# ChrisDud0257/SSL

Measured on AMD Instinct MI355X. Metric: SSG-loss edge-pixels/sec (fwd+bwd) 3x256x256 k_s=25 k_w=9, higher is better.
Workload: dtype f32; 1 GPU; C2: batch 16 x 3x256x256 per GPU, Laplacian mask, k_s=25 k_w=9 sigma=1.0, L1+KL w=1e3, SSGs materialised; launch=per-kernel, ranks_seen=1, edge_px_rank0=76466, images_rank0=16, input_checksum=c1391ff6908574f6, gradient_accumulation=fixed-point integer atomics (bit-reproducible, the shipped default), prewarm_steps=1949, parallelism=images sharded x1, no data-path collective

## Files before the change

### ssl_amd/csrc/ssg_dense.hip

```cpp
#include "ssg_host.hpp"

namespace ssg {

typedef float f2 __attribute__((ext_vector_type(2)));

template <int D>
__device__ __forceinline__ float quad_next(float v) {
  constexpr int ctrl = D == 1 ? 0xF9 : 0xFE;
  return __builtin_bit_cast(float, __builtin_amdgcn_update_dpp(0, __builtin_bit_cast(int, v), ctrl, 0xf, 0xf, true));
}

template <int LO, int LEN, typename T, int N>
__device__ __forceinline__ T block_sum(const T (&e)[N]) {
  static_assert(LEN >= 1 && (LEN & (LEN - 1)) == 0 && LO >= 0 && LO + LEN <= N, "power-of-two block inside the array");
  if constexpr (LEN == 1) return e[LO];
  else return block_sum<LO, LEN / 2>(e) + block_sum<LO + LEN / 2, LEN / 2>(e);
}
constexpr int floor_pow2(int n) { return n < 2 ? 1 : 2 * floor_pow2(n / 2); }
template <int LO, int LEN, typename T, int N>
__device__ __forceinline__ T sum_from(const T (&e)[N]) {
  constexpr int B = floor_pow2(LEN);
  if constexpr (B == LEN) return block_sum<LO, LEN>(e);
  else return block_sum<LO, B>(e) + sum_from<LO + B, LEN - B>(e);
}
template <int HI, int LEN, typename T, int N>
__device__ __forceinline__ T sum_upto(const T (&e)[N]) {
  constexpr int B = floor_pow2(LEN);
  if constexpr (B == LEN) return block_sum<HI - LEN, LEN>(e);
  else return block_sum<HI - B, B>(e) + sum_upto<HI - B, LEN - B>(e);
}

template <int KW>
__device__ __forceinline__ float tap_sum(const float (&v)[KW], const float (&w)[KW], float rest) {
  static_assert(KW % 2 == 1 && KW >= 5, "pairs of taps and a last one");
  constexpr int NP = KW / 2;
  f2 a = f2{v[0], v[1]} * f2{w[0], w[1]}, b = f2{v[2], v[3]} * f2{w[2], w[3]};
#pragma unroll
  for (int j = 2; j < NP; ++j) {
    const f2 vv = f2{v[2 * j], v[2 * j + 1]}, ww = f2{w[2 * j], w[2 * j + 1]};
    if (j % 2 == 0) a = __builtin_elementwise_fma(vv, ww, a);
    else b = __builtin_elementwise_fma(vv, ww, b);
  }
  const f2 r2 = a + b;
  return (r2.x + r2.y) + __builtin_fmaf(w[KW - 1], v[KW - 1], rest);
}

constexpr int DT_X = 32;
constexpr int dense_lane_px(int kw) { return kw == 9 ? 10 : 12; }
constexpr bool dense_h_paired(int kw) { return kw == 9; }
constexpr int dense_h_group(int kw) { return kw == 9 ? 10 : 12; }
constexpr int dense_h_stride(int kw) { return kw == 9 ? 40 : 49; }
__device__ __forceinline__ int dense_h_col(int ex, int L, int G, bool paired) {
  const int k = ex % L;
  return paired ? G * (ex / L) + 2 * (k % (L / 2)) + k / (L / 2) : ex;
}

template <int KS, int KW, int C, int NW, bool TM = false, bool RAW = false, int NCH = 0>
__device__ __forceinline__ void fwd_dense_body(const DenseParams &p) {
  static_assert(!(TM && RAW), "raw distances go to the caller's row-major rows");
  constexpr int NT = 64 * NW;
  constexpr int HP = KS / 2, HK = KW / 2, P = KS * KS, HALO = HP + HK, DT_Y = 16 - 2 * HK;
  constexpr int RH = DT_Y + 2 * HALO, RWD = DT_X + 2 * HALO, RS = RWD + 1;
  constexpr int UH = DT_Y + 2 * HK, UW = DT_X + 2 * HK;
  constexpr int L = dense_lane_px(KW), HL = L / 2;
  constexpr int NV = HL + KW - 1;
  constexpr int DT_HS = dense_h_stride(KW);
  constexpr bool HPAIR = dense_h_paired(KW);
  constexpr int HG = dense_h_group(KW);
  constexpr int NE_MAX = DT_Y * DT_X, NCHUNK = NCH > 0 ? NCH : NE_MAX / 64;
  constexpr bool PIPE = dense_h_paired(KW) && NCH > 0 && NCH <= 2 && !TM;
  static_assert(NCH == 0 || (dense_h_paired(KW) && NCH * 64 <= NE_MAX), "chunk classes exist for the 8 x 32 tiles only");
  static_assert(!TM || !HPAIR, "tile-major rows use the k_w 13 pixel map");
  static_assert(UH == 16 && DT_X == 32 && 4 * L >= UW && 3 * HG + L <= DT_HS && HG >= L && (HPAIR || HG == L) && L % 2 == 0 && KW - 1 <= L,
                "lane map: 16 U-rows x 4 column groups (one quad) of L pixels; a window spans two lanes");

  extern __shared__ __attribute__((aligned(16))) float smem[];
  float *reg = smem;
  float *F = reg + C * RH * RS;
  float *HF = F + UH * UW;
  float *Hb = HF + UH * DT_HS;
  double *rsum = (double *)Hb;
  constexpr int RSTR = UH * DT_HS / 2;
  static_assert(NE_MAX <= RSTR, "row sums alias the wave's H buffer");
  int *elist = (int *)(Hb + NW * UH * DT_HS);
  int *misc = elist + NE_MAX * 3;

  const int tid = threadIdx.x, lane = tid & 63, wv = tid >> 6;
  const int tslot = blockIdx.x / p.nimg, which = blockIdx.x - tslot * p.nimg;
  if (tslot >= dense_tile_count(p.n_dense)) return;
  if (p.tm_slots > 0 && tm_active(p.n_dense, p.tm_slots, rows_to_do(p.n_dev, p.n_host)) != TM) return;
  if (TM && p.tm_slots <= 0) return;
  if (p.n_dense[1] != DT_Y) {
    if (p.status && tid == 0) atomicOr(p.status, 1);
    return;
  }
  const int H = p.H, W = p.W;
  const int tx_n = (W + DT_X - 1) / DT_X, ty_n = (H + DT_Y - 1) / DT_Y;
  const int listed = dense_tile_at(p.n_dense, p.tiles, p.B * ty_n * tx_n, tslot);
  if (TM && p.strips && (listed & TILE_IN_STRIP)) return;
  if constexpr (NCH > 0) {
    if (((listed & TILE_HUGE) != 0) != (NCH > 2)) return;
  }
  const int tile = dense_tile_id(listed);
  const int b = tile / (tx_n * ty_n), tr = tile - b * tx_n * ty_n;
  const int ty0 = (tr / tx_n) * DT_Y, tx0 = (tr % tx_n) * DT_X;
  const int nrows = rows_to_do(p.n_dev, p.n_host);

  constexpr int CPLF = (RWD + 15) / 16, RPP = NT / 16, NPASS = (C * RH + RPP - 1) / RPP;
  const int lx = tid % 16, lr = tid / 16;
  int rank_px = -1;
  if constexpr (HPAIR) {
    const int y = ty0 + tid / DT_X, x = tx0 + tid % DT_X;
    const int v = p.rank[((size_t)b * H + (y < H ? y : H - 1)) * W + (x < W ? x : W - 1)];
    rank_px = (y < H && x < W) ? v : -1;
  }
  float rv[NPASS][CPLF];
  int rdst[NPASS];
  {
    const float *src = p.img[which] + (size_t)b * C * H * W;
#pragma unroll
    for (int h = 0; h < NPASS; ++h) {
      const int R = h * RPP + lr;
      const bool on = R < C * RH;
      const int Rc = on ? R : 0;
      const int c = Rc / RH, ry = Rc - c * RH;
      int gy = reflect_idx(ty0 - HALO + ry, H);
      gy = gy < 0 ? 0 : (gy >= H ? H - 1 : gy);
      const float *srow = src + ((size_t)c * H + gy) * W;
      rdst[h] = on ? (c * RH + ry) * RS : -1;
#pragma unroll
      for (int k = 0; k < CPLF; ++k) {
        int gx = reflect_idx(tx0 - HALO + lx + 16 * k, W);
        gx = gx < 0 ? 0 : (gx >= W ? W - 1 : gx);
        rv[h][k] = srow[gx];
      }
    }
  }
  if constexpr (HPAIR) {
    static_assert(DT_Y * DT_X == NT, "one thread per tile pixel");
    int *wcnt = misc + 16, *bstart = wcnt + NW * 32;
    const int ey = tid / DT_X, ex = tid % DT_X;
    int r = rank_px;
    if (r >= nrows) r = -1;
    elist[3 * tid + 2] = -1;
    const int bank = (DT_HS * ey + dense_h_col(ex, L, HG, true)) & 31;
    int pib = 0, mycnt = 0;
    for (int bk = 0; bk < 32; ++bk) {
      const unsigned long long m = __ballot(r >= 0 && bank == bk);
      if (bank == bk) pib = __popcll(m & ((1ull << lane) - 1ull));
      if (lane == bk) mycnt = __popcll(m);
    }
    if (lane < 32) wcnt[wv * 32 + lane] = mycnt;
    __syncthreads();
    if (tid < 32) {
      int c[NW], tot = 0;
#pragma unroll
      for (int k = 0; k < NW; ++k) {
        c[k] = wcnt[k * 32 + tid];
        tot += c[k];
      }
      int incl = tot;
#pragma unroll
      for (int o = 1; o < 32; o <<= 1) {
        const int t = __shfl_up(incl, o, 32);
        if (tid >= o) incl += t;
      }
      int run = incl - tot;
#pragma unroll
      for (int k = 0; k < NW; ++k) {
        bstart[k * 32 + tid] = run;
        run += c[k];
      }
      if (tid == 31) misc[NW] = 32 * ((incl + 31) / 32);
    }
    __syncthreads();
    if (r >= 0) {
      const int ng = misc[NW] / 32, i = bstart[wv * 32 + bank] + pib;
      const int pos = (i % ng) * 32 + i / ng;
      elist[3 * pos + 0] = ey;
      elist[3 * pos + 1] = ex;
      elist[3 * pos + 2] = r;
    }
  } else {
    static_assert(HPAIR || (DT_Y == 4 && NCHUNK == 2), "pair map: 4 x 32 tile, two pixels per lane");
    if (tid < NE_MAX) {
      const int pp = tid >> 6, ln = tid & 63;
      const int ey = 2 * (ln >> 5) + pp, ex = ln & 31;
      const int y = ty0 + ey, x = tx0 + ex;
      int r = (y < H && x < W) ? p.rank[((size_t)b * H + y) * W + x] : -1;
      if (r >= nrows) r = -1;
      elist[3 * tid + 0] = ey;
      elist[3 * tid + 1] = ex;
      elist[3 * tid + 2] = r;
    }
    if (tid == 0) misc[NW] = NE_MAX;
  }
#pragma unroll
  for (int h = 0; h < NPASS; ++h)
#pragma unroll
    for (int k = 0; k < CPLF; ++k)
      if (rdst[h] >= 0 && lx + 16 * k < RWD) reg[rdst[h] + lx + 16 * k] = rv[h][k];
  __syncthreads();
  const int n_e = misc[NW];
  for (int i = tid; i < UH * UW; i += NT) {
    const int ur = i / UW, uc = i - ur * UW;
    float t = 0.f;
#pragma unroll
    for (int c = 0; c < C; ++c) {
      const float v = reg[(c * RH + ur + HP) * RS + uc + HP];
      t = __builtin_fmaf(v, v, t);
    }
    F[i] = t;
  }
  __syncthreads();
  for (int i = tid; i < UH * DT_X; i += NT) {
    const int ur = i / DT_X, tc = i - ur * DT_X;
    float t = 0.f;
#pragma unroll
    for (int kx = 0; kx < KW; ++kx) t += F[ur * UW + tc + kx];
    HF[ur * DT_HS + dense_h_col(tc, L, HG, HPAIR)] = t;
  }
  __syncthreads();

  const int r = lane >> 2, g = lane & 3;
  f2 iu[C][HL];
#pragma unroll
  for (int c = 0; c < C; ++c)
#pragma unroll
    for (int j = 0; j < HL; ++j) {
      const float *q = reg + (c * RH + r + HP) * RS + L * g + HP + j;
      iu[c][j] = f2{q[0], q[HL]};
    }
  f2 Fv[NV];
#pragma unroll
  for (int m = 0; m < NV; ++m) {
    const int c0 = L * g + m, c1 = c0 + HL;
    Fv[m] = f2{F[r * UW + (c0 < UW ? c0 : UW - 1)], F[r * UW + (c1 < UW ? c1 : UW - 1)]};
  }
  float *hb = Hb + wv * UH * DT_HS;
  float *hrow = hb + r * DT_HS + HG * g;
  const float nk = (float)(-1.4426950408889634 / ((double)(C * KW * KW) * (double)p.sigma));
  double rs[NCHUNK];
#pragma unroll
  for (int k = 0; k < NCHUNK; ++k) rs[k] = 0.0;
  float *outp = p.out[which];
  int hoff[NCHUNK];
  size_t orow[NCHUNK];
  bool eon[NCHUNK];
#pragma unroll
  for (int ck = 0; ck < NCHUNK; ++ck) {
    const int e = ck * 64 + lane;
    eon[ck] = e < n_e && elist[3 * (e < n_e ? e : 0) + 2] >= 0;
    const int ec = (eon[ck] || !HPAIR) ? e : 0;
    const int ey = elist[3 * ec], ex = elist[3 * ec + 1];
    hoff[ck] = ey * DT_HS + dense_h_col(ex, L, HG, HPAIR);
    orow[ck] = eon[ck] ? (size_t)elist[3 * ec + 2] * P : 0;
  }

  const int n_e_stage = SSG_DBG(p, 2) ? 0 : n_e;
  const bool do_store = !SSG_DBG(p, 1);
  constexpr int SB = (KS == 49 && !TM) ? 7 : 13;
  constexpr int REM = (NCHUNK <= 2) ? KS % NW : 0;
  static_assert(REM == 0 || (REM == 1 && NW == 4 && KS > SB && KS <= 2 * SB), "one shared row, four runs: two store groups halved");
  constexpr int RUN1 = (SB + 1) / 2, RUN3 = SB + (KS - SB) / 2;
  const int wvu = __builtin_amdgcn_readfirstlane(wv);
  const int run_lo = wvu == 0 ? 0 : wvu == 1 ? RUN1 : wvu == 2 ? SB : RUN3;
  const int run_hi = wvu == 0 ? RUN1 : wvu == 1 ? SB : wvu == 2 ? RUN3 : KS;
  auto do_row = [&](const int qyi, auto shared_c, auto nact_c) {
    constexpr bool shared_row = decltype(shared_c)::value;
    constexpr int NACT = decltype(nact_c)::value;
    const int ylo = (-HK > -qyi) ? -HK : -qyi, yhi = (HK < KS - 1 - qyi) ? HK : KS - 1 - qyi;
    float wgt[KW];
#pragma unroll
    for (int k = 0; k < KW; ++k) wgt[k] = (k - HK >= ylo && k - HK <= yhi) ? 1.f : 0.f;
    const bool interior = ylo == -HK && yhi == HK;
    float av[NCHUNK];
#pragma unroll
    for (int ck = 0; ck < NCHUNK; ++ck) {
      av[ck] = 0.f;
      if (ck * 64 < n_e && (ylo > -HK || yhi < HK)) {
        const float *fc = HF + hoff[ck];
        float fv[KW], cw[KW];
#pragma unroll
        for (int k = 0; k < KW; ++k) {
          fv[k] = fc[k * DT_HS];
          cw[k] = 1.f - wgt[k];
        }
        av[ck] = tap_sum<KW>(fv, cw, 0.f);
      }
    }
    const float *rq = reg + (r + qyi) * RS + L * g;
    f2 w[C][HL];
    auto fill_window = [&](auto sc) {
      constexpr int S0 = decltype(sc)::value;
#pragma unroll
      for (int c = 0; c < C; ++c)
#pragma unroll
        for (int a = 0; a < L; ++a) {
          const float v = rq[c * RH * RS + ((a - S0) % L + L) % L + S0];
          if (a < HL) w[c][a].x = v;
          else w[c][a - HL].y = v;
        }
    };
    if constexpr (!shared_row) {
      fill_window(std::integral_constant<int, 0>{});
    } else {
      if (run_lo == 0) fill_window(std::integral_constant<int, 0>{});
      else if (run_lo == RUN1) fill_window(std::integral_constant<int, RUN1>{});
      else if (run_lo == SB) fill_window(std::integral_constant<int, SB>{});
      else fill_window(std::integral_constant<int, RUN3>{});
    }
    float evb[TM ? 1 : NCHUNK][TM ? 1 : SB];
    float *tmq = nullptr;
    if constexpr (TM) tmq = p.tm[which] + ((size_t)tslot * P + (size_t)qyi * KS) * (size_t)NE_MAX + lane;
    float hvp[PIPE ? NCHUNK : 1][KW];
    auto step = [&](auto qc, auto split_c) {
      constexpr int qxi = decltype(qc)::value;
      constexpr bool SPLIT = decltype(split_c)::value;
      constexpr int xlo = (-HK > -qxi) ? -HK : -qxi, xhi = (HK < KS - 1 - qxi) ? HK : KS - 1 - qxi;
      f2 E[HL];
      if constexpr (NCHUNK <= 2) {
#pragma unroll
        for (int c = 0; c < C; ++c) {
#pragma unroll
          for (int j = 0; j < HL; ++j) {
            const int a = (j + qxi) % L;
            const f2 wv2 = a < HL ? w[c][a] : w[c][a - HL].yx;
            const f2 d = iu[c][j] - wv2;
            E[j] = c == 0 ? d * d : __builtin_elementwise_fma(d, d, E[j]);
          }
        }
      } else {
#pragma unroll
        for (int j = 0; j < HL; ++j) {
          const int a = (j + qxi) % L;
          f2 t = f2{0.f, 0.f};
#pragma unroll
          for (int c = 0; c < C; ++c) {
            const f2 wv2 = a < HL ? w[c][a] : w[c][a - HL].yx;
            const f2 d = iu[c][j] - wv2;
            t = __builtin_elementwise_fma(d, d, t);
          }
          E[j] = t;
        }
      }
      f2 Hs[HL];
      if constexpr (xlo == -HK && xhi == HK) {
        float Pf[L], Sf[L];
        static_for(std::make_integer_sequence<int, HL>{}, [&](auto mc) {
          constexpr int m = decltype(mc)::value;
          const f2 pl = sum_from<0, m + 1>(E);
          const f2 su = sum_upto<HL, HL - m>(E);
          const f2 tot = sum_from<0, HL>(E);
          Pf[m] = pl.x;
          Pf[m + HL] = tot.x + pl.y;
          Sf[m + HL] = su.y;
          Sf[m] = su.x + tot.y;
        });
        float hs[L];
        if constexpr (KW == 9 && L == 10) {
          hs[0] = Pf[KW - 1];
#pragma unroll
          for (int k = 1; k < L; ++k) hs[k] = Sf[k];
          asm volatile("s_nop 1\n\t"
                       "v_add_f32_dpp %0, %8, %0 quad_perm:[1,2,3,3] row_mask:0xf bank_mask:0xf bound_ctrl:1\n\t"
                       "v_add_f32_dpp %1, %9, %1 quad_perm:[1,2,3,3] row_mask:0xf bank_mask:0xf bound_ctrl:1\n\t"
                       "v_add_f32_dpp %2, %10, %2 quad_perm:[1,2,3,3] row_mask:0xf bank_mask:0xf bound_ctrl:1\n\t"
                       "v_add_f32_dpp %3, %11, %3 quad_perm:[1,2,3,3] row_mask:0xf bank_mask:0xf bound_ctrl:1\n\t"
                       "v_add_f32_dpp %4, %12, %4 quad_perm:[1,2,3,3] row_mask:0xf bank_mask:0xf bound_ctrl:1\n\t"
                       "v_add_f32_dpp %5, %13, %5 quad_perm:[1,2,3,3] row_mask:0xf bank_mask:0xf bound_ctrl:1\n\t"
                       "v_add_f32_dpp %6, %14, %6 quad_perm:[1,2,3,3] row_mask:0xf bank_mask:0xf bound_ctrl:1\n\t"
                       "v_add_f32_dpp %7, %15, %7 quad_perm:[1,2,3,3] row_mask:0xf bank_mask:0xf bound_ctrl:1"
                       : "+v"(hs[2]), "+v"(hs[3]), "+v"(hs[4]), "+v"(hs[5]), "+v"(hs[6]), "+v"(hs[7]), "+v"(hs[8]), "+v"(hs[9])
                       : "v"(Pf[0]), "v"(Pf[1]), "v"(Pf[2]), "v"(Pf[3]), "v"(Pf[4]), "v"(Pf[5]), "v"(Pf[6]), "v"(Pf[7]));
        } else {
        static_for(std::make_integer_sequence<int, L>{}, [&](auto kc) {
          constexpr int k = decltype(kc)::value, last = k + KW - 1;
          if constexpr (last < L) {
            static_assert(k == 0 || last == L - 1, "in-lane windows: a prefix or a suffix");
            hs[k] = k == 0 ? Pf[last] : Sf[k];
          } else {
            hs[k] = Sf[k] + quad_next<1>(Pf[last - L]);
          }
        });
        }
#pragma unroll
        for (int k = 0; k < HL; ++k) Hs[k] = f2{hs[k], hs[k + HL]};
      } else {
        f2 V[NV];
#pragma unroll
        for (int m = 0; m < NV; ++m) {
          if (m < HL) V[m] = E[m];
          else if (m < L) V[m] = f2{E[m - HL].y, quad_next<1>(E[m - HL].x)};
          else V[m] = f2{quad_next<1>(E[m - L].x), quad_next<1>(E[m - L].y)};
        }
#pragma unroll
        for (int k = 0; k < HL; ++k) {
          f2 t = f2{0.f, 0.f};
          bool first = true;
#pragma unroll
          for (int tp = 0; tp < KW; ++tp) {
            const bool kept = tp - HK >= xlo && tp - HK <= xhi;
            const f2 v = kept ? V[k + tp] : Fv[k + tp];
            t = first ? v : t + v;
            first = false;
          }
          Hs[k] = t;
        }
      }
      if constexpr (HPAIR) {
#pragma unroll
        for (int k = 0; k < HL; ++k) *(f2 *)(hrow + 2 * k) = Hs[k];
      } else {
#pragma unroll
        for (int k = 0; k < HL; ++k) {
          hrow[k] = Hs[k].x;
          hrow[k + HL] = Hs[k].y;
        }
      }
      if (qxi + 1 < KS) {
        constexpr int sl = qxi % L;
#pragma unroll
        for (int c = 0; c < C; ++c) {
          const float v = rq[c * RH * RS + L + qxi];
          if constexpr (sl < HL) w[c][sl].x = v;
          else w[c][sl - HL].y = v;
        }
      }
      float dpair[2];
      if constexpr (!HPAIR) {
        if (n_e_stage > 0) {
          const float *hc = hb + hoff[0];
          float hv[KW + 1];
#pragma unroll
          for (int k = 0; k <= KW; ++k) hv[k] = hc[k * DT_HS];
          if (interior) {
            f2 t01 = f2{hv[2], hv[3]} + f2{hv[4], hv[5]}, t23 = f2{hv[6], hv[7]} + f2{hv[8], hv[9]};
            t01 = t01 + f2{hv[10], hv[11]};
            t01 = t01 + t23;
            const float common = (t01.x + t01.y) + (hv[1] + hv[KW - 1]);
            dpair[0] = common + hv[0];
            dpair[1] = common + hv[KW];
          } else {
            float h0[KW], h1[KW];
#pragma unroll
            for (int k = 0; k < KW; ++k) {
              h0[k] = hv[k];
              h1[k] = hv[k + 1];
            }
            dpair[0] = tap_sum<KW>(h0, wgt, av[0]);
            dpair[1] = tap_sum<KW>(h1, wgt, av[1]);
          }
        }
      }
      auto edge_gather = [&](int ck, float (&hv)[KW]) {
        const float *hc = hb + hoff[ck];
#pragma unroll
        for (int k = 0; k < KW; ++k) hv[k] = hc[k * DT_HS];
      };
      auto edge_emit = [&](auto qe_c, int ck, float d) {
        constexpr int QE = decltype(qe_c)::value;
          float ev;
          if constexpr (RAW) {
            ev = d;
          } else {
            ev = __builtin_amdgcn_exp2f(d * nk);
            rs[ck] += (double)ev;
            asm volatile("" : "+v"(rs[ck]));
          }
          if constexpr (TM) {
            if (do_store) tmq[QE * NE_MAX + ck * 64] = ev;
          } else {
          evb[ck][QE % SB] = ev;
          if (eon[ck] && do_store) {
            float *o = outp + orow[ck] + qyi * KS;
            constexpr bool ends = SPLIT ? (QE + 1 == RUN1 || QE + 1 == SB || QE + 1 == RUN3 || QE + 1 == KS)
                                        : (QE % SB == SB - 1 || QE == KS - 1);
            if constexpr (ends) {
              constexpr int q0 = !SPLIT ? QE - QE % SB : (QE + 1 == RUN1 ? 0 : QE + 1 == SB ? RUN1 : QE + 1 == RUN3 ? SB : RUN3);
              constexpr int cnt = QE + 1 - q0, i0 = q0 % SB;
#pragma unroll
              for (int t = 0; t + 4 <= cnt; t += 4) {
                float4 v4 = make_float4(evb[ck][i0 + t], evb[ck][i0 + t + 1], evb[ck][i0 + t + 2], evb[ck][i0 + t + 3]);
                if constexpr (RAW) {
                  float4 old;
                  __builtin_memcpy(&old, o + q0 + t, 16);
                  v4.x += old.x; v4.y += old.y; v4.z += old.z; v4.w += old.w;
                }
                __builtin_memcpy(o + q0 + t, &v4, 16);
              }
#pragma unroll
              for (int t = cnt & ~3; t < cnt; ++t) {
                if constexpr (RAW) o[q0 + t] += evb[ck][i0 + t];
                else o[q0 + t] = evb[ck][i0 + t];
              }
            }
          }
          }
      };
#pragma unroll
      for (int ck = 0; ck < (NACT >= 0 ? NACT : NCHUNK); ++ck) {
        if (NACT >= 0 || ck * 64 < n_e_stage) {
          if constexpr (PIPE && !SPLIT) {
            if constexpr (qxi > 0) edge_emit(std::integral_constant<int, qxi - 1>{}, ck, tap_sum<KW>(hvp[ck], wgt, av[ck]));
            edge_gather(ck, hvp[ck]);
            if constexpr (qxi == KS - 1) edge_emit(std::integral_constant<int, KS - 1>{}, ck, tap_sum<KW>(hvp[ck], wgt, av[ck]));
          } else if constexpr (HPAIR) {
            float hv[KW];
            edge_gather(ck, hv);
            edge_emit(std::integral_constant<int, qxi>{}, ck, tap_sum<KW>(hv, wgt, av[ck]));
          } else {
            edge_emit(std::integral_constant<int, qxi>{}, ck, dpair[ck]);
          }
        }
      }
    };
    if constexpr (!shared_row) {
      static_for(std::make_integer_sequence<int, KS>{}, [&](auto qc) { step(qc, std::false_type{}); });
    } else {
      static_for(std::make_integer_sequence<int, KS>{}, [&](auto qc) {
        constexpr int qxi = decltype(qc)::value;
        if (qxi >= run_lo && qxi < run_hi) step(qc, std::true_type{});
      });
    }
  };
  if (!SSG_DBG(p, 64)) {
#define SSG_ALL_ROWS(NACT_)                                                                                    \
  do {                                                                                                         \
    _Pragma("unroll 1") for (int qyi = wv; qyi < KS - REM; qyi += NW)                                          \
        do_row(qyi, std::false_type{}, std::integral_constant<int, NACT_>{});                                  \
    if constexpr (REM > 0) do_row(KS - 1, std::true_type{}, std::integral_constant<int, NACT_>{});             \
  } while (0)
    if constexpr (PIPE && NCHUNK == 2 && !RAW) {
      if (n_e_stage > 64) SSG_ALL_ROWS(2);
      else if (n_e_stage > 0) SSG_ALL_ROWS(1);
#ifdef SSG_PROFILE
      else SSG_ALL_ROWS(0);
#endif
    } else {
      SSG_ALL_ROWS(-1);
    }
#undef SSG_ALL_ROWS
  }

#pragma unroll
  for (int ck = 0; ck < NCHUNK; ++ck)
    if (ck * 64 + lane < n_e) rsum[wv * RSTR + ck * 64 + lane] = rs[ck];
  __threadfence_block();
  __syncthreads();
  if (RAW || !p.generalization || SSG_DBG(p, 8)) return;
  if (p.row_scale) {
    double *rsc = p.row_scale + (size_t)which * p.n_host;
    for (int e = tid; e < n_e; e += NT) {
      if (elist[3 * e + 2] < 0) continue;
      double tot = 0.0;
#pragma unroll
      for (int k = 0; k < NW; ++k) tot += rsum[k * RSTR + e];
      const double sc = 1.0 / (tot + (double)p.eps);
      rsc[elist[3 * e + 2]] = TM ? -sc : sc;
    }
    return;
  }
  if constexpr (TM) return;
  asm volatile("s_waitcnt vmcnt(0)" ::: "memory");
  __syncthreads();
  constexpr int RPL = (P + 63) / 64;
  for (int e0 = 2 * wv; e0 < n_e; e0 += 2 * NW) {
    float v[2][RPL];
    double scale[2];
    float *o[2];
    bool ok[2];
#pragma unroll
    for (int j = 0; j < 2; ++j) {
      const int e = e0 + j < n_e ? e0 + j : e0;
      ok[j] = e0 + j < n_e && elist[3 * e + 2] >= 0;
      double tot = 0.0;
#pragma unroll
      for (int k = 0; k < NW; ++k) tot += rsum[k * RSTR + e];
      scale[j] = 1.0 / (tot + (double)p.eps);
      o[j] = outp + (size_t)(ok[j] ? elist[3 * e + 2] : 0) * P;
#pragma unroll
      for (int k = 0; k < RPL; ++k) {
        const int q = lane + 64 * k;
        v[j][k] = q < P ? __builtin_nontemporal_load(o[j] + q) : 0.f;
      }
    }
#pragma unroll
    for (int j = 0; j < 2; ++j) {
      if (ok[j]) {
#pragma unroll
        for (int k = 0; k < RPL; ++k) {
          const int q = lane + 64 * k;
          if (q < P) o[j][q] = (float)(scale[j] * (double)v[j][k]);
        }
      }
    }
  }
}

template <int KS, int KW, int C, int NW, bool TM = false, bool RAW = false, int NCH = 0>
__global__ __launch_bounds__(64 * NW) __attribute__((amdgpu_waves_per_eu(2, 2))) void ssg_fwd_dense(DenseParams p) {
  fwd_dense_body<KS, KW, C, NW, TM, RAW, NCH>(p);
}

template <int KS, int KW, int C, int NW, bool RAW>
__global__ __launch_bounds__(64 * NW) __attribute__((amdgpu_waves_per_eu(2, 2))) void ssg_fwd_dense_classes(DenseParams p) {
  const int tslot = blockIdx.x / p.nimg;
  if (tslot >= dense_tile_count(p.n_dense)) return;
  const int tx_n = (p.W + DT_X - 1) / DT_X, ty_n = (p.H + 7) / 8;
  const int listed = dense_tile_at(p.n_dense, p.tiles, p.B * ty_n * tx_n, tslot);
  if (__builtin_amdgcn_readfirstlane(listed) & TILE_HUGE) fwd_dense_body<KS, KW, C, NW, false, RAW, 4>(p);
  else fwd_dense_body<KS, KW, C, NW, false, RAW, 2>(p);
}


#ifdef SSG_PROFILE
__device__ unsigned long long g_strip_times[3 * 1024];
#endif
template <int KS, int KW, int C, int NW>
__global__ __launch_bounds__(256 * NW) __attribute__((amdgpu_waves_per_eu(3, 3))) void ssg_fwd_strip(DenseParams p) {
#ifdef SSG_PROFILE
  if (threadIdx.x == 0 && blockIdx.x < 1024) {
    g_strip_times[3 * blockIdx.x] = __builtin_readcyclecounter();
    unsigned hwid, xcc;
    asm volatile("s_getreg_b32 %0, hwreg(HW_REG_HW_ID)" : "=s"(hwid));
    asm volatile("s_getreg_b32 %0, hwreg(HW_REG_XCC_ID)" : "=s"(xcc));
    g_strip_times[3 * blockIdx.x + 2] = ((unsigned long long)xcc << 32) | hwid;
  }
#endif
  constexpr int NT = 128 * NW, NTR = 64 * NW;
  constexpr int HP = KS / 2, HK = KW / 2, P = KS * KS, HALO = HP + HK;
  constexpr int UH = 16 * NW, SY = UH - 2 * HK;
  constexpr int RWD = DT_X + 2 * HALO, RS = RWD + 1;
  constexpr int UW = DT_X + 2 * HK;
  constexpr int L = dense_lane_px(KW), HL = L / 2, NV = HL + KW - 1;
  constexpr int HS = DT_X + 1;
  constexpr int PX = SY * DT_X / NTR, NHV = PX + KW - 1;
  static_assert(SY == STRIP_ROWS && SY * DT_X == PX * NTR && NTR % DT_X == 0 && (NTR / DT_X) * PX == SY && 4 * L >= UW && L % 2 == 0 &&
                KW - 1 <= L && KW == 13 && PX == 6, "lane maps: 16 U-rows per wave, 6 centres of a column per lane");

  constexpr int STRIP_LDS = C * UH * RS + 3 * UH * HS + UH * UW + 16;
  extern __shared__ __attribute__((aligned(16))) float smem_wg[];
  const int half = threadIdx.x / NT;
  float *smem = smem_wg + half * STRIP_LDS;
  float *band = smem;
  float *HF = band + C * UH * RS;
  float *Hb = HF + UH * HS;
  float *F = Hb + 2 * UH * HS;

  const int tid = threadIdx.x - half * NT, lane = tid & 63, wv = tid >> 6;
  const int n_act = p.strips[0] < p.max_strips ? p.strips[0] : p.max_strips, n_jobs = n_act * p.nimg;
  if (2 * (int)blockIdx.x >= n_jobs) return;
  const int job = 2 * (int)blockIdx.x + half < n_jobs ? 2 * (int)blockIdx.x + half : n_jobs - 1;
  const int which = job / n_act, slot = job - which * n_act;
  const int nrows = rows_to_do(p.n_dev, p.n_host);
  if (!tm_active(p.n_dense, p.tm_slots, nrows)) return;
  const int H = p.H, W = p.W;
  const int tx_n = (W + DT_X - 1) / DT_X, sy_n = (H + SY - 1) / SY;
  const int strip = p.strips[1 + 2 * slot], first = p.strips[2 + 2 * slot];
  const int b = strip / (tx_n * sy_n), tr = strip - b * tx_n * sy_n;
  const int ty0 = (tr / tx_n) * SY, tx0 = (tr % tx_n) * DT_X;
  const float *src = p.img[which] + (size_t)b * C * H * W;
  auto lds_barrier = [] { asm volatile("s_waitcnt lgkmcnt(0)\n\ts_barrier" ::: "memory"); };

  auto fill_band = [&](int rho0) {
    constexpr int CPLF = (RWD + 15) / 16, RPP = NT / 16;
    const int lx = tid % 16, lr = tid / 16;
    for (int R0 = 0; R0 < C * UH; R0 += RPP) {
      const int R = R0 + lr;
      const int c = R / UH, i = R - c * UH, rho = rho0 + i;
      int gy = reflect_idx(ty0 - HALO + rho, H);
      gy = gy < 0 ? 0 : (gy >= H ? H - 1 : gy);
      const float *srow = src + ((size_t)c * H + gy) * W;
      float v[CPLF];
#pragma unroll
      for (int k = 0; k < CPLF; ++k) {
        int gx = reflect_idx(tx0 - HALO + lx + 16 * k, W);
        gx = gx < 0 ? 0 : (gx >= W ? W - 1 : gx);
        v[k] = srow[gx];
      }
      float *drow = band + (c * UH + rho % UH) * RS;
#pragma unroll
      for (int k = 0; k < CPLF; ++k)
        if (lx + 16 * k < RWD) drow[lx + 16 * k] = v[k];
    }
  };
  static_assert((C * UH) % (NT / 16) == 0, "whole row passes");

  fill_band(HP);
  __syncthreads();
  const bool eh_role = wv < NW;
  const int r = lane >> 2, g = lane & 3, R = 16 * (eh_role ? wv : 0) + r;
  f2 iu[C][HL];
#pragma unroll
  for (int c = 0; c < C; ++c)
#pragma unroll
    for (int j = 0; j < HL; ++j) {
      const float *q = band + (c * UH + (R + HP) % UH) * RS + L * g + HP + j;
      iu[c][j] = f2{q[0], q[HL]};
    }
  for (int i = tid; i < UH * UW; i += NT) {
    const int ur = i / UW, uc = i - ur * UW;
    float t = 0.f;
#pragma unroll
    for (int c = 0; c < C; ++c) {
      const float v = band[(c * UH + (ur + HP) % UH) * RS + uc + HP];
      t = __builtin_fmaf(v, v, t);
    }
    F[i] = t;
  }
  __syncthreads();
  for (int i = tid; i < UH * DT_X; i += NT) {
    const int ur = i / DT_X, tc = i - ur * DT_X;
    float t = 0.f;
#pragma unroll
    for (int kx = 0; kx < KW; ++kx) t += F[ur * UW + tc + kx];
    HF[ur * HS + tc] = t;
  }
  const int frow_off = R * UW + (g < 3 ? L * g : UW - NV - HL);
  __syncthreads();
  fill_band(0);

  const int tid_e = eh_role ? 0 : tid - NTR;
  const int ecol = tid_e % DT_X, e0 = (tid_e / DT_X) * PX;
  const int ty_n = (H + 3) / 4, n_tq = ty_n - ty0 / 4 < SY / 4 ? ty_n - ty0 / 4 : SY / 4;
  int orow[PX];
  unsigned coff[PX];
  float *const tmbase = __builtin_amdgcn_readfirstlane(which) ? p.tm[1] : p.tm[0];
#pragma unroll
  for (int j = 0; j < PX; ++j) {
    const int y = ty0 + e0 + j, x = tx0 + ecol;
    const int rk = (y < H && x < W) ? p.rank[((size_t)b * H + y) * W + x] : -1;
    orow[j] = rk >= nrows ? -1 : rk;
    const int tq = (e0 + j) >> 2, ey = (e0 + j) & 3;
    coff[j] = (unsigned)(tq < n_tq ? first + tq : p.tm_slots) * (unsigned)(P * TM_PX) + (unsigned)(64 * (ey & 1) + 32 * (ey >> 1) + ecol);
  }
  int pf_gx = reflect_idx(tx0 - HALO + (tid < RWD ? tid : 0), W);
  pf_gx = pf_gx < 0 ? 0 : (pf_gx >= W ? W - 1 : pf_gx);
  const float nk = (float)(-1.4426950408889634 / ((double)(C * KW * KW) * (double)p.sigma));
  double rs[PX];
#pragma unroll
  for (int j = 0; j < PX; ++j) rs[j] = 0.0;
  float *hwrite = Hb + R * HS + L * g;
  constexpr int HSPLIT = DT_X - 2 * L, GA = 2, GB = 1;
  static_assert(L == 12 && DT_X == 32 && HSPLIT == 8, "groups 0, 1 whole, group 2 its first eight centres, group 3 none");
  const float *hread = Hb + e0 * HS + ecol;
  const float *hfread = HF + e0 * HS + ecol;
  __syncthreads();

  if (eh_role) __builtin_amdgcn_s_setprio(1);
  if (eh_role) {
#pragma unroll 1
  for (int qyi = 0; qyi < KS; ++qyi) {
    float pf[C];
    if (qyi + 1 < KS && tid < RWD) {
      int gy = reflect_idx(ty0 - HALO + qyi + UH, H);
      gy = gy < 0 ? 0 : (gy >= H ? H - 1 : gy);
#pragma unroll
      for (int c = 0; c < C; ++c) pf[c] = src[((size_t)c * H + gy) * W + pf_gx];
    }
    const float *rq = band + ((R + qyi) % UH) * RS + L * g;
    f2 w[C][HL];
#pragma unroll
    for (int c = 0; c < C; ++c)
#pragma unroll
      for (int t = 0; t < HL; ++t) w[c][t] = f2{rq[c * UH * RS + t], rq[c * UH * RS + t + HL]};
    float *hw_even = hwrite + (qyi & 1) * UH * HS, *hw_odd = hwrite + ((qyi & 1) ^ 1) * UH * HS;
    auto eh_stage = [&](auto qc) {
      constexpr int qxi = decltype(qc)::value;
      constexpr int xlo = (-HK > -qxi) ? -HK : -qxi, xhi = (HK < KS - 1 - qxi) ? HK : KS - 1 - qxi;
      f2 E[HL];
#pragma unroll
      for (int j = 0; j < HL; ++j) {
        const int a = (j + qxi) % L;
        f2 t = f2{0.f, 0.f};
#pragma unroll
        for (int c = 0; c < C; ++c) {
          const f2 wv2 = a < HL ? w[c][a] : w[c][a - HL].yx;
          const f2 d = iu[c][j] - wv2;
          t = __builtin_elementwise_fma(d, d, t);
        }
        E[j] = t;
      }
      float hs[L];
      if constexpr (xlo == -HK && xhi == HK) {
        float Pf[L], Sf[L];
        static_for(std::make_integer_sequence<int, HL>{}, [&](auto mc) {
          constexpr int m = decltype(mc)::value;
          const f2 pl = sum_from<0, m + 1>(E);
          const f2 su = sum_upto<HL, HL - m>(E);
          const f2 tot = sum_from<0, HL>(E);
          Pf[m] = pl.x;
          Pf[m + HL] = tot.x + pl.y;
          Sf[m + HL] = su.y;
          Sf[m] = su.x + tot.y;
        });
        static_assert(KW - 1 >= L && L == 12, "all twelve windows reach into the next lane");
#pragma unroll
        for (int k = 0; k < L; ++k) hs[k] = Sf[k];
        asm volatile("s_nop 1\n\t"
                     "v_add_f32_dpp %0, %6, %0 quad_perm:[1,2,3,3] row_mask:0xf bank_mask:0xf bound_ctrl:1\n\t"
                     "v_add_f32_dpp %1, %7, %1 quad_perm:[1,2,3,3] row_mask:0xf bank_mask:0xf bound_ctrl:1\n\t"
                     "v_add_f32_dpp %2, %8, %2 quad_perm:[1,2,3,3] row_mask:0xf bank_mask:0xf bound_ctrl:1\n\t"
                     "v_add_f32_dpp %3, %9, %3 quad_perm:[1,2,3,3] row_mask:0xf bank_mask:0xf bound_ctrl:1\n\t"
                     "v_add_f32_dpp %4, %10, %4 quad_perm:[1,2,3,3] row_mask:0xf bank_mask:0xf bound_ctrl:1\n\t"
                     "v_add_f32_dpp %5, %11, %5 quad_perm:[1,2,3,3] row_mask:0xf bank_mask:0xf bound_ctrl:1"
                     : "+v"(hs[0]), "+v"(hs[1]), "+v"(hs[2]), "+v"(hs[3]), "+v"(hs[4]), "+v"(hs[5])
                     : "v"(Pf[0]), "v"(Pf[1]), "v"(Pf[2]), "v"(Pf[3]), "v"(Pf[4]), "v"(Pf[5]));
        asm volatile("s_nop 1\n\t"
                     "v_add_f32_dpp %0, %6, %0 quad_perm:[1,2,3,3] row_mask:0xf bank_mask:0xf bound_ctrl:1\n\t"
                     "v_add_f32_dpp %1, %7, %1 quad_perm:[1,2,3,3] row_mask:0xf bank_mask:0xf bound_ctrl:1\n\t"
                     "v_add_f32_dpp %2, %8, %2 quad_perm:[1,2,3,3] row_mask:0xf bank_mask:0xf bound_ctrl:1\n\t"
                     "v_add_f32_dpp %3, %9, %3 quad_perm:[1,2,3,3] row_mask:0xf bank_mask:0xf bound_ctrl:1\n\t"
                     "v_add_f32_dpp %4, %10, %4 quad_perm:[1,2,3,3] row_mask:0xf bank_mask:0xf bound_ctrl:1\n\t"
                     "v_add_f32_dpp %5, %11, %5 quad_perm:[1,2,3,3] row_mask:0xf bank_mask:0xf bound_ctrl:1"
                     : "+v"(hs[6]), "+v"(hs[7]), "+v"(hs[8]), "+v"(hs[9]), "+v"(hs[10]), "+v"(hs[11])
                     : "v"(Pf[6]), "v"(Pf[7]), "v"(Pf[8]), "v"(Pf[9]), "v"(Pf[10]), "v"(Pf[11]));
      } else {
        int fo = frow_off;
        asm volatile("" : "+v"(fo));
        const float *frow = F + fo;
        f2 V[NV];
#pragma unroll
        for (int m = 0; m < NV; ++m) {
          if (m < HL) V[m] = E[m];
          else if (m < L) V[m] = f2{E[m - HL].y, quad_next<1>(E[m - HL].x)};
          else V[m] = f2{quad_next<1>(E[m - L].x), quad_next<1>(E[m - L].y)};
        }
#pragma unroll
        for (int k = 0; k < HL; ++k) {
          f2 t = f2{0.f, 0.f};
          bool first_tap = true;
#pragma unroll
          for (int tp = 0; tp < KW; ++tp) {
            const bool kept = tp - HK >= xlo && tp - HK <= xhi;
            const f2 v = kept ? V[k + tp] : f2{frow[k + tp], frow[k + tp + HL]};
            t = first_tap ? v : t + v;
            first_tap = false;
          }
          hs[k] = t.x;
          hs[k + HL] = t.y;
        }
      }
      float *hw = qxi % 2 == 0 ? hw_even : hw_odd;
      if (SSG_DBG(p, 32)) {
#pragma unroll
        for (int k = 0; k < L; ++k) asm volatile("" ::"v"(hs[k]));
      } else {
        if (g <= GA) {
#pragma unroll
          for (int k = 0; k < HSPLIT; ++k) hw[k] = hs[k];
        }
        if (g <= GB) {
#pragma unroll
          for (int k = HSPLIT; k < L; ++k) hw[k] = hs[k];
        }
      }
      if (qxi + 1 < KS && !SSG_DBG(p, 128)) {
        constexpr int sl = qxi % L;
#pragma unroll
        for (int c = 0; c < C; ++c) {
          const float v = rq[c * UH * RS + L + qxi];
          if constexpr (sl < HL) w[c][sl].x = v;
          else w[c][sl - HL].y = v;
        }
      }
    };
    if (!SSG_DBG(p, 4)) eh_stage(std::integral_constant<int, 0>{});
    lds_barrier();
    static_for(std::make_integer_sequence<int, KS - 1>{}, [&](auto qc) {
      if (!SSG_DBG(p, 4)) eh_stage(std::integral_constant<int, decltype(qc)::value + 1>{});
      lds_barrier();
    });
    if (qyi + 1 < KS) {
      if (tid < RWD) {
#pragma unroll
        for (int c = 0; c < C; ++c) band[(c * UH + qyi % UH) * RS + tid] = pf[c];
      }
      lds_barrier();
    }
  }
  } else {
#pragma unroll 1
  for (int qyi = 0; qyi < KS; ++qyi) {
    const int ylo = (-HK > -qyi) ? -HK : -qyi, yhi = (HK < KS - 1 - qyi) ? HK : KS - 1 - qyi;
    float wgt[KW];
#pragma unroll
    for (int k = 0; k < KW; ++k)
      wgt[k] = __builtin_bit_cast(float, __builtin_amdgcn_readfirstlane((k - HK >= ylo && k - HK <= yhi) ? 0x3f800000 : 0));
    const bool interior = ylo == -HK && yhi == HK;
    float av[PX];
#pragma unroll
    for (int j = 0; j < PX; ++j) av[j] = 0.f;
    if (!interior) {
      float hf[NHV], cw[KW];
#pragma unroll
      for (int t = 0; t < NHV; ++t) hf[t] = hfread[t * HS];
#pragma unroll
      for (int k = 0; k < KW; ++k) cw[k] = 1.f - wgt[k];
#pragma unroll
      for (int j = 0; j < PX; ++j) {
        float fv[KW];
#pragma unroll
        for (int k = 0; k < KW; ++k) fv[k] = hf[j + k];
        av[j] = tap_sum<KW>(fv, cw, 0.f);
      }
    }
    const float *hr_even = hread + (qyi & 1) * UH * HS, *hr_odd = hread + ((qyi & 1) ^ 1) * UH * HS;
    static_assert(NHV == 18, "nine pairs");
    f2 P[NHV / 2];
    auto h_requests = [&](auto qc) {
      constexpr int qxi = decltype(qc)::value;
      const float *hc = qxi % 2 == 0 ? hr_even : hr_odd;
      if (SSG_DBG(p, 16)) return;
#pragma unroll
      for (int m = 0; m < NHV / 2; ++m) P[m] = f2{hc[2 * m * HS], hc[(2 * m + 1) * HS]};
    };
    auto edge_stage = [&](auto qc) {
      constexpr int qxi = decltype(qc)::value;
      float d[PX];
      if (interior) {
        f2 T[8], Q[4];
#pragma unroll
        for (int m = 0; m < 8; ++m) T[m] = P[m] + P[m + 1];
#pragma unroll
        for (int a = 0; a < 4; ++a) Q[a] = (T[a] + T[a + 2]) + T[a + 4];
        float S[4];
#pragma unroll
        for (int a = 0; a < 4; ++a) S[a] = Q[a].x + Q[a].y;
#pragma unroll
        for (int a = 0; a < 3; ++a) {
          d[2 * a] = S[a] + P[a + 6].x;
          d[2 * a + 1] = P[a].y + S[a + 1];
        }
      } else {
        f2 we[6], wo[6];
#pragma unroll
        for (int m = 0; m < 6; ++m) {
          we[m] = f2{wgt[2 * m], wgt[2 * m + 1]};
          wo[m] = f2{wgt[2 * m + 1], wgt[2 * m + 2]};
        }
#pragma unroll
        for (int a = 0; a < 3; ++a) {
          f2 e0 = P[a] * we[0], e1 = P[a + 1] * we[1];
          f2 o0 = P[a + 1] * wo[0], o1 = P[a + 2] * wo[1];
#pragma unroll
          for (int m = 2; m < 6; ++m) {
            if (m % 2 == 0) {
              e0 = __builtin_elementwise_fma(P[a + m], we[m], e0);
              o0 = __builtin_elementwise_fma(P[a + 1 + m], wo[m], o0);
            } else {
              e1 = __builtin_elementwise_fma(P[a + m], we[m], e1);
              o1 = __builtin_elementwise_fma(P[a + 1 + m], wo[m], o1);
            }
          }
          const f2 e = e0 + e1, o = o0 + o1;
          d[2 * a] = (e.x + e.y) + __builtin_fmaf(wgt[12], P[a + 6].x, av[2 * a]);
          d[2 * a + 1] = (o.x + o.y) + __builtin_fmaf(wgt[0], P[a].y, av[2 * a + 1]);
        }
      }
      if (SSG_DBG(p, 8)) {
#pragma unroll
        for (int j = 0; j < PX; ++j) asm volatile("" ::"v"(d[j]));
      } else
#pragma unroll
      for (int j = 0; j < PX; ++j) {
        const float ev = __builtin_amdgcn_exp2f(d[j] * nk);
        rs[j] += (double)ev;
        asm volatile("" : "+v"(rs[j]));
        if (!SSG_DBG(p, 1)) (tmbase + (size_t)(qyi * KS + qxi) * TM_PX)[coff[j]] = ev;
      }
    };
    lds_barrier();
    h_requests(std::integral_constant<int, 0>{});
    static_for(std::make_integer_sequence<int, KS>{}, [&](auto qc) {
      constexpr int qxi = decltype(qc)::value;
      if (!SSG_DBG(p, 2)) edge_stage(qc);
      if constexpr (qxi + 1 < KS) {
        lds_barrier();
        if (!SSG_DBG(p, 2)) h_requests(std::integral_constant<int, qxi + 1>{});
      }
    });
    if (qyi + 1 < KS) lds_barrier();
  }
  }
#ifdef SSG_PROFILE
  if (threadIdx.x == 0 && blockIdx.x < 1024) g_strip_times[3 * blockIdx.x + 1] = __builtin_readcyclecounter();
#endif
  double *rsc = p.row_scale + (size_t)which * p.n_host;
  if (!eh_role) {
#pragma unroll
    for (int j = 0; j < PX; ++j)
      if (orow[j] >= 0) rsc[orow[j]] = -1.0 / (rs[j] + (double)p.eps);
  }
}

template <int KS, int KW, int C, int NW>
static size_t dense_lds_bytes() {
  constexpr int DT_Y = 16 - 2 * (KW / 2);
  constexpr int HALO = KS / 2 + KW / 2, RH = DT_Y + 2 * HALO, RS = DT_X + 2 * HALO + 1;
  constexpr int UH = DT_Y + 2 * (KW / 2), UW = DT_X + 2 * (KW / 2), NE = DT_Y * DT_X, DT_HS = dense_h_stride(KW);
  return sizeof(float) * (size_t)(C * RH * RS + UH * UW + UH * DT_HS + NW * UH * DT_HS) + sizeof(int) * (NE * 3 + 16 + 64 * NW);
}

bool dense_supported(int ks, int kw, int C) { return C == 3 && ((ks == 25 && kw == 9) || (ks == 49 && kw == 13)); }

int dense_tile_rows(int ks) { return ks == 49 ? 4 : 8; }

int dense_max_tiles(int B, int H, int W, int ks) {
  const int ty = dense_tile_rows(ks);
  return B * ((H + ty - 1) / ty) * ((W + DT_X - 1) / DT_X);
}

template <int KS, int KW, int C, int NW, bool TM, bool RAW = false, int NCH = 0>
static int launch_fwd_dense_t(DenseParams p, int n_tiles, hipStream_t st) {
  if (n_tiles <= 0) return 0;
  const size_t lds = dense_lds_bytes<KS, KW, C, NW>();
  static std::atomic<unsigned long long> lds_set{0};
  if (const int rc = ensure_dynamic_lds(ssg_fwd_dense<KS, KW, C, NW, TM, RAW, NCH>, (int)lds, lds_set)) return rc;
  p.grid_tiles = n_tiles;
  hipLaunchKernelGGL((ssg_fwd_dense<KS, KW, C, NW, TM, RAW, NCH>), dim3((unsigned)n_tiles * p.nimg), dim3(64 * NW), lds, st, p);
  return (int)hipGetLastError();
}

template <bool RAW>
static int launch_fwd_dense_25(const DenseParams &p0, hipStream_t st) {
  static const bool one_launch = env_int("SSG_DENSE_ONE_LAUNCH", 1) != 0;
  if (one_launch) {
    DenseParams p = p0;
    if (p.max_tiles <= 0) return 0;
    const size_t lds = dense_lds_bytes<25, 9, 3, 4>();
    static std::atomic<unsigned long long> lds_set{0};
    if (const int rc = ensure_dynamic_lds(ssg_fwd_dense_classes<25, 9, 3, 4, RAW>, (int)lds, lds_set)) return rc;
    p.grid_tiles = p.max_tiles;
    hipLaunchKernelGGL((ssg_fwd_dense_classes<25, 9, 3, 4, RAW>), dim3((unsigned)p.max_tiles * p.nimg), dim3(256), lds, st, p);
    return (int)hipGetLastError();
  }
  const DenseParams &p = p0;
  int rc = launch_fwd_dense_t<25, 9, 3, 4, false, RAW, 2>(p, p.max_tiles, st);
  const int heavy_max = p.n_host / 65 + 1;
  if (!rc) rc = launch_fwd_dense_t<25, 9, 3, 4, false, RAW, 4>(p, heavy_max < p.max_tiles ? heavy_max : p.max_tiles, st);
  return rc;
}

int dense_max_strips(int B, int H, int W, int ks) {
  return ks == 49 ? B * ((H + STRIP_ROWS - 1) / STRIP_ROWS) * ((W + DT_X - 1) / DT_X) : 0;
}

template <int KS, int KW, int C, int NW>
static int launch_fwd_strip_t(const DenseParams &p, hipStream_t st) {
  constexpr int UH = 16 * NW, HALO = KS / 2 + KW / 2, RS = DT_X + 2 * HALO + 1, HS = DT_X + 1;
  const size_t lds = sizeof(float) * (size_t)(C * UH * RS + 3 * UH * HS + UH * (DT_X + KW - 1) + 16);
  static std::atomic<unsigned long long> lds_set{0};
  if (const int rc = ensure_dynamic_lds(ssg_fwd_strip<KS, KW, C, NW>, 2 * (int)lds, lds_set)) return rc;
  hipLaunchKernelGGL((ssg_fwd_strip<KS, KW, C, NW>), dim3((unsigned)(p.max_strips * p.nimg + 1) / 2), dim3(256 * NW), 2 * lds, st, p);
  return (int)hipGetLastError();
}

#ifdef SSG_PROFILE
int strip_times(unsigned long long *host, int n) {
  return (int)hipMemcpyFromSymbol(host, HIP_SYMBOL(g_strip_times), sizeof(unsigned long long) * (size_t)(n < 3072 ? n : 3072));
}
int strip_occupancy() {
  constexpr int KS = 49, KW = 13, C = 3, NW = 3, UH = 16 * NW, HALO = KS / 2 + KW / 2, RS = DT_X + 2 * HALO + 1, HS = DT_X + 1;
  const size_t lds = sizeof(float) * (size_t)(C * UH * RS + 3 * UH * HS + UH * (DT_X + KW - 1) + 16);
  static std::atomic<unsigned long long> lds_set{0};
  if (ensure_dynamic_lds(ssg_fwd_strip<KS, KW, C, NW>, 2 * (int)lds, lds_set)) return -1;
  int n = -1;
  if (hipOccupancyMaxActiveBlocksPerMultiprocessor(&n, ssg_fwd_strip<KS, KW, C, NW>, 256 * NW, 2 * lds) != hipSuccess) return -2;
  return n;
}
#endif

int launch_fwd_dense(const DenseParams &p0, int ks, int kw, int C, hipStream_t st) {
  if (!dense_supported(ks, kw, C)) return -1;
  if (p0.max_tiles == 0) return 0;
  DenseParams p = p0;
  const bool tm = ks == 49 && p.tm[0] && p.tm_slots > 0 && p.row_scale && p.generalization && (p.nimg == 1 || p.tm[1]);
  if (!tm) p.tm_slots = 0;
  if (p.raw) {
    p.tm_slots = 0;
    p.row_scale = nullptr;
    p.strips = nullptr;
    if (ks == 25) return launch_fwd_dense_25<true>(p, st);
    return launch_fwd_dense_t<49, 13, 3, 7, false, true>(p, p.max_tiles, st);
  }
  if (ks == 25) return launch_fwd_dense_25<false>(p, st);
  if (!tm) p.strips = nullptr;
  int rc = (tm && p.strips && p.max_strips > 0) ? launch_fwd_strip_t<49, 13, 3, 3>(p, st) : 0;
  if (!rc && tm) rc = launch_fwd_dense_t<49, 13, 3, 7, true>(p, p.tm_slots < p.max_tiles ? p.tm_slots : p.max_tiles, st);
  if (!rc) rc = launch_fwd_dense_t<49, 13, 3, 7, false>(p, p.max_tiles, st);
  return rc;
}

}
```

Baseline: 66.70 million edge-px/s.

## Store per-wave H rows lane-major with ds_write_addtid and hoist previous tap sums

For k_w=9, the per-wave horizontal-sum buffer moves from a row-major, pair-interleaved layout to a lane-indexed block layout. Each of the 10 per-lane outputs lands in its own block, written with ds_write_addtid_b32 through inline asm with m0 set to the wave's buffer base. Edge gathers now read with a tap stride of 4 and use block offsets picked to spread LDS banks. The previous step's tap_sum is also computed before the H store, so its arithmetic can overlap the LDS writes. This shrinks the buffer and cuts store instruction overhead, but relies on inline asm and a hand-tuned bank map.

Measured after the change: 66.94 million edge-px/s, median of 6. No clear change (+0.4%).

```diff
diff --git a/ssl_amd/csrc/ssg_dense.hip b/ssl_amd/csrc/ssg_dense.hip
--- a/ssl_amd/csrc/ssg_dense.hip
+++ b/ssl_amd/csrc/ssg_dense.hip
@@ -47,12 +47,43 @@
 
 constexpr int DT_X = 32;
 constexpr int dense_lane_px(int kw) { return kw == 9 ? 10 : 12; }
-constexpr bool dense_h_paired(int kw) { return kw == 9; }
-constexpr int dense_h_group(int kw) { return kw == 9 ? 10 : 12; }
-constexpr int dense_h_stride(int kw) { return kw == 9 ? 40 : 49; }
-__device__ __forceinline__ int dense_h_col(int ex, int L, int G, bool paired) {
-  const int k = ex % L;
-  return paired ? G * (ex / L) + 2 * (k % (L / 2)) + k / (L / 2) : ex;
+constexpr bool dense_h_by_lane(int kw) { return kw == 9; }
+constexpr int dense_h_stride(int kw) { return 49; }
+constexpr int dense_hl_block(int k) {
+  constexpr int B[10] = {0, 402, 135, 471, 336, 269, 202, 68, 605, 538};
+  return B[k];
+}
+constexpr int DENSE_HL_TAP = 4;
+constexpr int dense_h_size(int kw) { return kw == 9 ? 670 : 16 * dense_h_stride(kw); }
+static_assert(dense_hl_block(8) + 64 <= dense_h_size(9) && dense_h_size(9) % 2 == 0, "the last block ends inside the buffer");
+__device__ __forceinline__ int dense_h_at(int ur, int tc, int kw) {
+  if (!dense_h_by_lane(kw)) return ur * dense_h_stride(kw) + tc;
+  const int L = dense_lane_px(9), g = tc / L;
+  return dense_hl_block(tc - L * g) + DENSE_HL_TAP * ur + g;
+}
+
+__device__ __forceinline__ void dense_h_store_by_lane(unsigned base, const float (&h)[10]) {
+#pragma clang diagnostic push
+#pragma clang diagnostic ignored "-Winline-asm"
+  asm volatile("s_mov_b32 m0, %10\n\t"
+               "s_nop 0\n\t"
+               "ds_write_addtid_b32 %0 offset:%11\n\t"
+               "ds_write_addtid_b32 %1 offset:%12\n\t"
+               "ds_write_addtid_b32 %2 offset:%13\n\t"
+               "ds_write_addtid_b32 %3 offset:%14\n\t"
+               "ds_write_addtid_b32 %4 offset:%15\n\t"
+               "ds_write_addtid_b32 %5 offset:%16\n\t"
+               "ds_write_addtid_b32 %6 offset:%17\n\t"
+               "ds_write_addtid_b32 %7 offset:%18\n\t"
+               "ds_write_addtid_b32 %8 offset:%19\n\t"
+               "ds_write_addtid_b32 %9 offset:%20"
+               :
+               : "v"(h[0]), "v"(h[1]), "v"(h[2]), "v"(h[3]), "v"(h[4]), "v"(h[5]), "v"(h[6]), "v"(h[7]), "v"(h[8]), "v"(h[9]),
+                 "s"(base), "n"(4 * dense_hl_block(0)), "n"(4 * dense_hl_block(1)), "n"(4 * dense_hl_block(2)),
+                 "n"(4 * dense_hl_block(3)), "n"(4 * dense_hl_block(4)), "n"(4 * dense_hl_block(5)), "n"(4 * dense_hl_block(6)),
+                 "n"(4 * dense_hl_block(7)), "n"(4 * dense_hl_block(8)), "n"(4 * dense_hl_block(9))
+               : "memory", "m0");
+#pragma clang diagnostic pop
 }
 
 template <int KS, int KW, int C, int NW, bool TM = false, bool RAW = false, int NCH = 0>
@@ -64,25 +95,25 @@
   constexpr int UH = DT_Y + 2 * HK, UW = DT_X + 2 * HK;
   constexpr int L = dense_lane_px(KW), HL = L / 2;
   constexpr int NV = HL + KW - 1;
-  constexpr int DT_HS = dense_h_stride(KW);
-  constexpr bool HPAIR = dense_h_paired(KW);
-  constexpr int HG = dense_h_group(KW);
+  constexpr bool HLANE = dense_h_by_lane(KW);
+  constexpr int DT_HS = dense_h_stride(KW), HB = dense_h_size(KW);
+  constexpr int TAP = HLANE ? DENSE_HL_TAP : DT_HS;
   constexpr int NE_MAX = DT_Y * DT_X, NCHUNK = NCH > 0 ? NCH : NE_MAX / 64;
-  constexpr bool PIPE = dense_h_paired(KW) && NCH > 0 && NCH <= 2 && !TM;
-  static_assert(NCH == 0 || (dense_h_paired(KW) && NCH * 64 <= NE_MAX), "chunk classes exist for the 8 x 32 tiles only");
-  static_assert(!TM || !HPAIR, "tile-major rows use the k_w 13 pixel map");
-  static_assert(UH == 16 && DT_X == 32 && 4 * L >= UW && 3 * HG + L <= DT_HS && HG >= L && (HPAIR || HG == L) && L % 2 == 0 && KW - 1 <= L,
+  constexpr bool PIPE = dense_h_by_lane(KW) && NCH > 0 && NCH <= 2 && !TM;
+  static_assert(NCH == 0 || (dense_h_by_lane(KW) && NCH * 64 <= NE_MAX), "chunk classes exist for the 8 x 32 tiles only");
+  static_assert(!TM || !HLANE, "tile-major rows use the k_w 13 pixel map");
+  static_assert(UH == 16 && DT_X == 32 && 4 * L >= UW && (HLANE || 4 * L <= DT_HS) && L % 2 == 0 && KW - 1 <= L,
                 "lane map: 16 U-rows x 4 column groups (one quad) of L pixels; a window spans two lanes");
 
   extern __shared__ __attribute__((aligned(16))) float smem[];
   float *reg = smem;
   float *F = reg + C * RH * RS;
   float *HF = F + UH * UW;
-  float *Hb = HF + UH * DT_HS;
+  float *Hb = HF + HB;
   double *rsum = (double *)Hb;
-  constexpr int RSTR = UH * DT_HS / 2;
-  static_assert(NE_MAX <= RSTR, "row sums alias the wave's H buffer");
-  int *elist = (int *)(Hb + NW * UH * DT_HS);
+  constexpr int RSTR = HB / 2;
+  static_assert(NE_MAX <= RSTR && HB % 2 == 0 && (C * RH * RS + UH * UW) % 2 == 0, "row sums alias the wave's H buffer, as doubles");
+  int *elist = (int *)(Hb + NW * HB);
   int *misc = elist + NE_MAX * 3;
 
   const int tid = threadIdx.x, lane = tid & 63, wv = tid >> 6;
@@ -109,7 +140,7 @@
   constexpr int CPLF = (RWD + 15) / 16, RPP = NT / 16, NPASS = (C * RH + RPP - 1) / RPP;
   const int lx = tid % 16, lr = tid / 16;
   int rank_px = -1;
-  if constexpr (HPAIR) {
+  if constexpr (HLANE) {
     const int y = ty0 + tid / DT_X, x = tx0 + tid % DT_X;
     const int v = p.rank[((size_t)b * H + (y < H ? y : H - 1)) * W + (x < W ? x : W - 1)];
     rank_px = (y < H && x < W) ? v : -1;
@@ -136,14 +167,14 @@
       }
     }
   }
-  if constexpr (HPAIR) {
+  if constexpr (HLANE) {
     static_assert(DT_Y * DT_X == NT, "one thread per tile pixel");
     int *wcnt = misc + 16, *bstart = wcnt + NW * 32;
     const int ey = tid / DT_X, ex = tid % DT_X;
     int r = rank_px;
     if (r >= nrows) r = -1;
     elist[3 * tid + 2] = -1;
-    const int bank = (DT_HS * ey + dense_h_col(ex, L, HG, true)) & 31;
+    const int bank = dense_h_at(ey, ex, KW) & 31;
     int pib = 0, mycnt = 0;
     for (int bk = 0; bk < 32; ++bk) {
       const unsigned long long m = __ballot(r >= 0 && bank == bk);
@@ -182,7 +213,7 @@
       elist[3 * pos + 2] = r;
     }
   } else {
-    static_assert(HPAIR || (DT_Y == 4 && NCHUNK == 2), "pair map: 4 x 32 tile, two pixels per lane");
+    static_assert(HLANE || (DT_Y == 4 && NCHUNK == 2), "pair map: 4 x 32 tile, two pixels per lane");
     if (tid < NE_MAX) {
       const int pp = tid >> 6, ln = tid & 63;
       const int ey = 2 * (ln >> 5) + pp, ex = ln & 31;
@@ -218,7 +249,7 @@
     float t = 0.f;
 #pragma unroll
     for (int kx = 0; kx < KW; ++kx) t += F[ur * UW + tc + kx];
-    HF[ur * DT_HS + dense_h_col(tc, L, HG, HPAIR)] = t;
+    HF[dense_h_at(ur, tc, KW)] = t;
   }
   __syncthreads();
 
@@ -237,8 +268,9 @@
     const int c0 = L * g + m, c1 = c0 + HL;
     Fv[m] = f2{F[r * UW + (c0 < UW ? c0 : UW - 1)], F[r * UW + (c1 < UW ? c1 : UW - 1)]};
   }
-  float *hb = Hb + wv * UH * DT_HS;
-  float *hrow = hb + r * DT_HS + HG * g;
+  float *hb = Hb + wv * HB;
+  float *hrow = hb + r * DT_HS + L * g;
+  const unsigned hb_lds = __builtin_amdgcn_readfirstlane((unsigned)(size_t)(__attribute__((address_space(3))) float *)hb);
   const float nk = (float)(-1.4426950408889634 / ((double)(C * KW * KW) * (double)p.sigma));
   double rs[NCHUNK];
 #pragma unroll
@@ -251,9 +283,9 @@
   for (int ck = 0; ck < NCHUNK; ++ck) {
     const int e = ck * 64 + lane;
     eon[ck] = e < n_e && elist[3 * (e < n_e ? e : 0) + 2] >= 0;
-    const int ec = (eon[ck] || !HPAIR) ? e : 0;
+    const int ec = (eon[ck] || !HLANE) ? e : 0;
     const int ey = elist[3 * ec], ex = elist[3 * ec + 1];
-    hoff[ck] = ey * DT_HS + dense_h_col(ex, L, HG, HPAIR);
+    hoff[ck] = dense_h_at(ey, ex, KW);
     orow[ck] = eon[ck] ? (size_t)elist[3 * ec + 2] * P : 0;
   }
 
@@ -283,7 +315,7 @@
         float fv[KW], cw[KW];
 #pragma unroll
         for (int k = 0; k < KW; ++k) {
-          fv[k] = fc[k * DT_HS];
+          fv[k] = fc[k * TAP];
           cw[k] = 1.f - wgt[k];
         }
         av[ck] = tap_sum<KW>(fv, cw, 0.f);
@@ -345,6 +377,7 @@
         }
       }
       f2 Hs[HL];
+      float ho[HLANE ? L : 1];
       if constexpr (xlo == -HK && xhi == HK) {
         float Pf[L], Sf[L];
         static_for(std::make_integer_sequence<int, HL>{}, [&](auto mc) {
@@ -384,8 +417,13 @@
           }
         });
         }
-#pragma unroll
-        for (int k = 0; k < HL; ++k) Hs[k] = f2{hs[k], hs[k + HL]};
+        if constexpr (HLANE) {
+#pragma unroll
+          for (int k = 0; k < L; ++k) ho[k] = hs[k];
+        } else {
+#pragma unroll
+          for (int k = 0; k < HL; ++k) Hs[k] = f2{hs[k], hs[k + HL]};
+        }
       } else {
         f2 V[NV];
 #pragma unroll
@@ -406,11 +444,25 @@
             first = false;
           }
           Hs[k] = t;
-        }
-      }
-      if constexpr (HPAIR) {
-#pragma unroll
-        for (int k = 0; k < HL; ++k) *(f2 *)(hrow + 2 * k) = Hs[k];
+          if constexpr (HLANE) {
+            ho[k] = t.x;
+            ho[k + HL] = t.y;
+          }
+        }
+      }
+      float dprev[PIPE ? NCHUNK : 1];
+      if constexpr (PIPE && !SPLIT && qxi > 0) {
+#pragma unroll
+        for (int ck = 0; ck < (NACT >= 0 ? NACT : NCHUNK); ++ck) {
+          dprev[ck] = 0.f;
+          if (NACT >= 0 || ck * 64 < n_e_stage) {
+            dprev[ck] = tap_sum<KW>(hvp[ck], wgt, av[ck]);
+            asm volatile("" : : "v"(dprev[ck]));
+          }
+        }
+      }
+      if constexpr (HLANE) {
+        dense_h_store_by_lane(hb_lds, ho);
       } else {
 #pragma unroll
         for (int k = 0; k < HL; ++k) {
@@ -428,7 +480,7 @@
         }
       }
       float dpair[2];
-      if constexpr (!HPAIR) {
+      if constexpr (!HLANE) {
         if (n_e_stage > 0) {
           const float *hc = hb + hoff[0];
           float hv[KW + 1];
@@ -456,7 +508,7 @@
       auto edge_gather = [&](int ck, float (&hv)[KW]) {
         const float *hc = hb + hoff[ck];
 #pragma unroll
-        for (int k = 0; k < KW; ++k) hv[k] = hc[k * DT_HS];
+        for (int k = 0; k < KW; ++k) hv[k] = hc[k * TAP];
       };
       auto edge_emit = [&](auto qe_c, int ck, float d) {
         constexpr int QE = decltype(qe_c)::value;
@@ -502,10 +554,10 @@
       for (int ck = 0; ck < (NACT >= 0 ? NACT : NCHUNK); ++ck) {
         if (NACT >= 0 || ck * 64 < n_e_stage) {
           if constexpr (PIPE && !SPLIT) {
-            if constexpr (qxi > 0) edge_emit(std::integral_constant<int, qxi - 1>{}, ck, tap_sum<KW>(hvp[ck], wgt, av[ck]));
+            if constexpr (qxi > 0) edge_emit(std::integral_constant<int, qxi - 1>{}, ck, dprev[ck]);
             edge_gather(ck, hvp[ck]);
             if constexpr (qxi == KS - 1) edge_emit(std::integral_constant<int, KS - 1>{}, ck, tap_sum<KW>(hvp[ck], wgt, av[ck]));
-          } else if constexpr (HPAIR) {
+          } else if constexpr (HLANE) {
             float hv[KW];
             edge_gather(ck, hv);
             edge_emit(std::integral_constant<int, qxi>{}, ck, tap_sum<KW>(hv, wgt, av[ck]));
@@ -999,8 +1051,8 @@
 static size_t dense_lds_bytes() {
   constexpr int DT_Y = 16 - 2 * (KW / 2);
   constexpr int HALO = KS / 2 + KW / 2, RH = DT_Y + 2 * HALO, RS = DT_X + 2 * HALO + 1;
-  constexpr int UH = DT_Y + 2 * (KW / 2), UW = DT_X + 2 * (KW / 2), NE = DT_Y * DT_X, DT_HS = dense_h_stride(KW);
-  return sizeof(float) * (size_t)(C * RH * RS + UH * UW + UH * DT_HS + NW * UH * DT_HS) + sizeof(int) * (NE * 3 + 16 + 64 * NW);
+  constexpr int UH = DT_Y + 2 * (KW / 2), UW = DT_X + 2 * (KW / 2), NE = DT_Y * DT_X, HB = dense_h_size(KW);
+  return sizeof(float) * (size_t)(C * RH * RS + UH * UW + HB + NW * HB) + sizeof(int) * (NE * 3 + 16 + 64 * NW);
 }
 
 bool dense_supported(int ks, int kw, int C) { return C == 3 && ((ks == 25 && kw == 9) || (ks == 49 && kw == 13)); }
```
